# nextpyp/pyp

Measured on AMD Instinct MI355X. Metric: particles/sec projection-matching, 256^2 box, higher is better.
Workload: dtype f32

## Files before the change

### pyp_amd/csrc/host_refine.h

```cpp
#pragma once

static int launch_prep(DevBuf<float2> &spill , const float *d_images, const double *d_rows, int n_img, const Geom &gm, double Rm_px, float fall_px,
                       int normalize, int invert, int do_mask, int whiten, float2 *band, float *wring,
                       const uint32_t *samples, int S_pad, float2 *Il, float *cw, float2 *Wp, float *C2, float *nI,
                       unsigned *band_max = nullptr ,
                       const float *focus_px = nullptr ) {
    if (int rc = ensure_plan(gm.N)) return rc;
    PrepP P;
    P.images = d_images; P.rows = d_rows; P.plan = g.plans[gm.N].plan;
    P.N = gm.N; P.B = gm.B; P.W = gm.W; P.H = gm.H;
    P.r_hi2 = (float)(gm.r_hi * gm.r_hi); P.Rm = (float)Rm_px; P.wfall = fall_px; P.a = (float)gm.a;
    P.Rm2_bg = (float)std::min(std::floor(Rm_px * Rm_px), 16777216.0);
    P.normalize = normalize; P.invert = invert; P.do_mask = do_mask; P.whiten = whiten;
    for (int k = 0; k < 4; k++) P.focus[k] = focus_px ? focus_px[k] : 0.f;
    P.band_max = band_max;
    P.band = band; P.wring = wring; P.samples = samples; P.S_pad = S_pad; P.Il = Il; P.cw = cw;
    P.Wp = Wp; P.C2 = C2; P.nI = nI; P.Bs = gm.Bs; P.Hs = gm.Hs;
    P.r_s2 = (float)(gm.r_s * gm.r_s); P.r_lo2 = (float)(gm.r_lo * gm.r_lo);
    const PrepPlan pl = prep_plan(gm.N, gm.B, gm.W);
    if (pl.err) return fail(-12, pl.err);
    P.L = pl.L; P.nc = pl.nc; P.nchunks = pl.nchunks; P.TS = pl.TS; P.WS = pl.WS;
    P.spill = nullptr;
    if (!pl.scratch_free) {
        if (int rc = spill.ensure((size_t)n_img * gm.N * gm.W)) return rc;
        P.spill = spill.p;
    }
    if (int rc = pl.scratch_free ? raise_lds_limit((const void *)k_prep<512, 2>, 160 * 1024) : raise_lds_limit((const void *)k_prep<256, 3>, 80 * 1024)) return rc;
    ProfScope ps(PPM_K_PREP);
    if (pl.scratch_free) hipLaunchKernelGGL((k_prep<512, 2>), dim3(n_img), dim3(512), pl.lds.total, cur_stream(), P);
    else hipLaunchKernelGGL((k_prep<256, 3>), dim3(n_img), dim3(256), pl.lds.total, cur_stream(), P);
    HIPCHK(hipGetLastError());
    return 0;
}

template <int... I>
static const void *global_kernel_at(int i, std::integer_sequence<int, I...>) {
    static const void *const fn[] = { (const void *)k_global<I / 4 + 1, (I & 2) != 0, (I & 1) != 0>... };
    return fn[i];
}
static const void *global_kernel(int R, bool half, int Bs) {
    const bool two = Bs <= 31;
    return global_kernel_at(((R >= 1 && R <= 5 ? R : 6) - 1) * 4 + (half ? 2 : 0) + (two ? 1 : 0), std::make_integer_sequence<int, 24>());
}
static size_t global_lds_bytes(int HsP, int n_orient, int R, int *topk_lds) {
    size_t lds = (size_t)HsP * 64 * sizeof(float2) * global_particles(R);
    if (lds < 1024) lds = 1024;
    const size_t lds_topk = (size_t)(32 + n_orient) * sizeof(float);
    const int fits = lds_topk <= (size_t)160 * 1024 ? 1 : 0;
    if (topk_lds) *topk_lds = fits;
    if (fits && lds_topk > lds) lds = lds_topk;
    return lds;
}
static int launch_global(GlobP &P, int n_img, bool half, int R) {
    P.n = n_img;
    const size_t lds = global_lds_bytes(P.HsP, P.n_orient, R, &P.topk_lds);
    const void *fn = global_kernel(R, half, P.Bs);
    if (int rc = raise_lds_limit(fn, 160 * 1024)) return rc;
    ProfScope ps(PPM_K_GLOBAL);
    const int ngroups = (n_img + global_particles(R) - 1) / global_particles(R);
    void *args[] = { &P };
    HIPCHK(hipLaunchKernel(fn, dim3(std::min(ngroups, g.cu_count)), dim3(global_threads(R)), args, lds, cur_stream()));
    return 0;
}

struct GfftPlan { int LN = 0, L = 0, RC = 0, nchunk = 1; size_t fixed = 0, t_bytes = 0, lds = 0; int topk_lds = 0; };
static bool gfft_plan(const Geom &gm, GfftPlan &pl) {
    int LN = 0; while ((1 << LN) < gm.Ns) LN++;
    if ((1 << LN) != gm.Ns || LN < 4 || LN > 7) return false;
    pl.LN = LN; pl.L = gm.Ns / 2;
    const int L = pl.L, G = gfft_slices_per_pass(L), NR = 2 * gm.RSy + 1;
    const size_t row = (size_t)G * 2 * gfft_row_stride(L) * sizeof(float2), fixed = (size_t)L * L * sizeof(float4) + gfft_small_bytes(L);
    const size_t room = (size_t)160 * 1024 - fixed;
    int RC = NR;
    if (const char *e = getenv("PPM_GFFT_ROWS")) { const int v = atoi(e); if (v > 0 && v < RC) RC = v; }
    if ((size_t)RC * row > room) RC = (int)(room / row);
    if (RC > 2 * L) RC = 2 * L;
    pl.RC = RC; pl.nchunk = (NR + RC - 1) / RC;
    pl.RC = (NR + pl.nchunk - 1) / pl.nchunk;
    pl.t_bytes = std::max((size_t)pl.RC * row, (size_t)G * L * L * sizeof(float4));
    pl.fixed = fixed;
    return true;
}
static void gfft_plan_topk(GfftPlan &pl, int n_orient) {
    const size_t topk = (size_t)n_orient * sizeof(float);
    pl.topk_lds = 0;
    if (topk <= pl.t_bytes) pl.topk_lds = 1;
    else if (pl.fixed + topk <= (size_t)160 * 1024) { pl.topk_lds = 1; pl.t_bytes = (topk + 15) & ~(size_t)15; }
    pl.lds = pl.fixed + pl.t_bytes;
}
static const void *gfft_kernel(int LN, bool chunked) {
    static const void *const fn[] = { (const void *)k_gfft<4, false>, (const void *)k_gfft<4, true>, (const void *)k_gfft<5, false>, (const void *)k_gfft<5, true>,
                                      (const void *)k_gfft<6, false>, (const void *)k_gfft<6, true>, (const void *)k_gfft<7, false>, (const void *)k_gfft<7, true> };
    return fn[((LN >= 4 && LN <= 6 ? LN : 7) - 4) * 2 + (chunked ? 1 : 0)];
}
static int launch_gfft(GfftP &P, int n_img, const GfftPlan &pl) {
    P.n = n_img; P.RC = pl.RC; P.nchunk = pl.nchunk; P.t_bytes = (int)pl.t_bytes; P.topk_lds = pl.topk_lds;
    const void *fn = gfft_kernel(pl.LN, pl.nchunk > 1);
    if (int rc = raise_lds_limit(fn, 160 * 1024)) return rc;
    ProfScope ps(PPM_K_GLOBAL);
    void *args[] = { &P };
    HIPCHK(hipLaunchKernel(fn, dim3(n_img), dim3(256), args, pl.lds, cur_stream()));
#ifdef PPM_GFFT_STAMPS
    {
        float st[4 * 4 * 12];
        HIPCHK(hipStreamSynchronize(cur_stream()));
        HIPCHK(hipMemcpy(st, P.cc, sizeof(st), hipMemcpyDeviceToHost));
        const char *names[12] = { "products", "fft", "stores", "barrier A", "row tail", "barrier B", "twiddles", "loop", "row reads + pairs", "row fft", "row max", "-" };
        const int nsl = P.n_dir * P.npsi_store;
        for (int b = 0; b < 4 && b < n_img; b++) for (int w = 0; w < 4; w++) {
            fprintf(stderr, "k_gfft stamps block %d wave %d (cycles per slice):", b, w);
            for (int i = 0; i < 11; i++) fprintf(stderr, " | %s %.0f", names[i], st[(b * 4 + w) * 12 + i] / nsl);
            fprintf(stderr, "\n");
        }
    }
#endif
    return 0;
}

static void launch_defocus(const CubeView &cv, const Geom &gm, const uint32_t *samples, int S_pad, const float2 *Il, const float *wring, const double *rows,
                           LState *states, int n, int nt, float step, float *ddef, double *all_scores, float rcls2) {
    const int nrings = gm.B + 2;
    DefocusP DP;
    DP.cv = cv; DP.samples = samples; DP.Il = Il; DP.wring = wring; DP.S_pad = S_pad; DP.nrings = nrings; DP.N = gm.N; DP.B = gm.B;
    DP.rlo2 = (float)(gm.r_lo * gm.r_lo); DP.rmax2 = (float)(gm.r_hi * gm.r_hi); DP.ring_signed = (float)std::min(gm.ring_signed, 1e30); DP.a = (float)gm.a;
    DP.rows = rows; DP.states = states; DP.ddef = ddef; DP.nt = nt; DP.step = step; DP.all_scores = all_scores; DP.rcls2 = rcls2;
    long knob = 0;
    if (const char *e = std::getenv("PPM_DEFOCUS_CHUNK")) knob = std::atol(e);
    DP.tchunk = ppm::defocus_chunk(nt, nrings, knob);
    ProfScope ps(PPM_K_LOCAL);
    hipLaunchKernelGGL(k_defocus, dim3(n), dim3(256), ring_lds_bytes(4, DP.tchunk, nrings), cur_stream(), DP);
}

namespace {
struct LocalLaunch { LocalP P = {}; int threads = 0, per_particle = 1; double evals = 0; bool near = false; };
struct RefineRun {
    ppm_ref *ref = nullptr; const ppm_refine_cfg *cfg = nullptr;
    Geom gm; SampleList sl; CubeView cv;
    int S_pad = 0, nrings = 0, CH = 0;
    int K = 0, Tb = 0, Tc = 0;
    double Rm_px = 0; float fall_px = 0;
    bool focus_on = false, sep_search = false; float focus_px[4] = { 0, 0, 0, 0 };
    GfftPlan gpl; bool use_fft = false;
    RowPlan rows = {};
    int Rtx = 0, Rty = 0, Rwin = 0, HsP = 0, nslices = 0; std::vector<int> cxs, cys;
    std::vector<GridSection> secs; std::vector<int> kpre; int sec_dirs = 0;
    LocalP base = {}; bool local_tab = false;
    double bf = 3.0; bool any_ang = false, any_sh = false;
    double ha0 = 0, hs0 = 0;
    int ndef = 0;
    int per_iter = 0; bool cls_on = false;
    LocalLaunch hit, fin;
    double sample_evals = 0;
    bool overlap = false; int tenants = 0;
    unsigned long long *reuse = nullptr;

    int ntiles() const { return (int)(cxs.size() * cys.size()); }
    int nsec() const { return (int)secs.size(); }
    size_t bank_slice() const { return (size_t)HsP * 64; }
    size_t bank4_slice() const { return use_fft ? (size_t)gpl.L * gpl.L : 0; }
    size_t HS() const { return (size_t)gm.Hs * 64; }
    int prefix_of(double rband) const { int rg = (int)std::ceil(rband); if (rg > gm.B + 1) rg = gm.B + 1; return sl.ring_off[rg]; }
    int reach_of(int S) const { int b = gm.B + 2; while (b > 1 && sl.ring_off[b] > S) b--; return std::min(gm.B, b - 1); }
};
constexpr int kTileR = 6;
constexpr int kFinalThreads = 256;
}

static void refine_notes(ppm_ref *ref, const ppm_refine_cfg *cfg, const Geom &gm) {
    ref->note.clear();
    if (gm.r_s_asked > gm.r_s) {
        char b[256];
        std::snprintf(b, sizeof(b), "NOTE: global search band lowered from %.1f to %.1f Fourier pixels (%.2f A instead of %.2f A): the grid-search "
                      "kernel covers 64 pixels; the top hits are refined up to the high-resolution limit as asked", gm.r_s_asked, gm.r_s,
                      gm.N * gm.a / gm.r_s, gm.N * gm.a / gm.r_s_asked);
        ref->note = b;
    }
    if (cfg->global_search && gm.range_capped) {
        char b[320];
        std::snprintf(b, sizeof(b), "%sNOTE: shift window of the grid search: +-%.0f x +-%.0f pixels (%d x %d search-grid steps of %.1f pixels, the most the "
                      "search grid of %d points holds; asked: %.0f pixels); the refinement of the hits is not limited to it", ref->note.empty() ? "" : "\n",
                      gm.RSx * gm.step, gm.RSy * gm.step, gm.RSx, gm.RSy, gm.step, gm.Ns, gm.range_asked_px);
        ref->note += b;
    }
}

static size_t workspace_budget() { return g.total_mem / 4; }
static size_t bank_budget() {
    size_t b = g.total_mem / 4;
    if (const char *e = std::getenv("PPM_BANK_BYTES")) { const long long v = std::atoll(e); if (v > 0 && (size_t)v < b) b = (size_t)v; }
    return b;
}

static int plan_grid_sections(RefineRun &r) {
    ppm_ref *ref = r.ref; const Geom &gm = r.gm;
    std::string err;
    const size_t budget = bank_budget();
    if (!plan_sections(gm.n_dir, gm.npsi_store, r.bank_slice() * sizeof(float2), r.bank4_slice() * sizeof(float4), budget, r.secs, err)) return fail(-22, err);
    if (r.nsec() > 1 && !r.use_fft && r.ntiles() > 1) {
        char b[320];
        std::snprintf(b, sizeof(b), "PPM_GLOBAL_PATH=tiles keeps the slice bank of the whole grid (%.2f GB at an angular step of %.3g degrees), the bank may take "
                      "%.2f GB; use a coarser angular step or the default path, which searches the grid in sections", (double)r.nslices * r.bank_slice() * sizeof(float2) / 1073741824.0,
                      gm.dstep, budget / 1073741824.0);
        return fail(-22, b);
// ... 706 lines not shown
```

### pyp_amd/csrc/ppm_kernels.h

```cpp
#pragma once
#include "ppm_dev.h"
#include "ppm_geom.h"
#include "ppm_rows.h"
#include "ppm_window.h"
#include <type_traits>

namespace ppm {

struct FftLinesP {
    float2 *data; FftPlan plan;
    int n, inverse, line_major, L;
    long nlines, inner, inner_stride, outer_stride, elem_stride;
};

__global__ void __launch_bounds__(256) k_fft_lines(FftLinesP P) {
    extern __shared__ __attribute__((aligned(16))) char smem[];
    __shared__ long lbase[16];
    __shared__ float2 tw_s[512];
    float2 *buf = (float2 *)smem;
    const int tid = threadIdx.x, n = P.n, LS = n + 1;
    long l0 = (long)blockIdx.x * P.L;
    int nl = (int)((P.nlines - l0) < P.L ? (P.nlines - l0) : P.L);
    if (nl <= 0) return;
    if (tid < nl) { const long l = l0 + tid; lbase[tid] = (l / P.inner) * P.outer_stride + (l % P.inner) * P.inner_stride; }
    for (int i = tid; i < n; i += 256) tw_s[i] = P.plan.tw[i];
    __syncthreads();
    const int dl = P.line_major ? 256 % nl : 256 / n, de = P.line_major ? 256 / nl : 256 % n;
    const int line0 = P.line_major ? tid % nl : tid / n, e0 = P.line_major ? tid / nl : tid % n;
    auto next = [&](int &line, int &e) {
        line += dl; e += de;
        if (P.line_major) { if (line >= nl) { line -= nl; e++; } } else if (e >= n) { e -= n; line++; }
    };
    {
        int line = line0, e = e0;
        for (int i = tid; i < nl * n; i += 256, next(line, e)) buf[line * LS + P.plan.perm[e]] = P.data[lbase[line] + e * P.elem_stride];
    }
    lds_fft(buf, P.plan, nl, LS, P.inverse != 0, tid, 256, tw_s);
    {
        int line = line0, e = e0;
        for (int i = tid; i < nl * n; i += 256, next(line, e)) P.data[lbase[line] + e * P.elem_stride] = buf[line * LS + e];
    }
}

__global__ void k_ref_load(const float *__restrict__ vol, float2 *__restrict__ f, int n, int np) {
    size_t i = (size_t)blockIdx.x * blockDim.x + threadIdx.x, n3 = (size_t)n * n * n;
    if (i >= n3) return;
    int x = (int)(i % n), y = (int)((i / n) % n), z = (int)(i / ((size_t)n * n));
    float g = 1.f;
    int c[3] = { x, y, z };
#pragma unroll
    for (int q = 0; q < 3; q++) {
        float u = kPiF * (float)(c[q] - n / 2) / (float)np;
        float sv = fabsf(u) < 1e-6f ? 1.f : sinf(u) / u;
        g *= 1.f / (sv * sv);
    }
    const int o0 = (np - n) / 2;
    f[((size_t)(z + o0) * np + (y + o0)) * np + (x + o0)] = make_float2(vol[i] * g, 0.f);
}

__global__ void k_ref_crop(const float2 *__restrict__ f, float2 *__restrict__ cube, int n, int n_orig, int B, int CX, int CY, int NBX, int NBY, unsigned LB,
                           const float *__restrict__ ringw, int nw) {
    size_t i = (size_t)blockIdx.x * blockDim.x + threadIdx.x, tot = (size_t)CX * CY * CY;
    if (i >= tot) return;
    const int x = (int)(i % CX), ys = (int)((i / CX) % CY), zs = (int)(i / ((size_t)CX * CY));
    const int y = ys - (B + 1), z = zs - (B + 1);
    int iz = ((z % n) + n) % n, iy = ((y % n) + n) % n, ix = x % n;
    float2 v = f[((size_t)iz * n + iy) * n + ix];
    float sg = (((x + y + z) & 1) ? -1.f : 1.f) / (float)n_orig;
    if (ringw) {
        const float kk = sqrtf((float)(x * x + y * y + z * z)) * (float)n_orig / (float)n;
        const int k0 = (int)kk;
        const float fr = kk - (float)k0;
        sg *= k0 + 1 < nw ? ringw[k0] + fr * (ringw[k0 + 1] - ringw[k0]) : ringw[nw - 1];
    }
    v = make_float2(v.x * sg, v.y * sg);
    cube[cube_element(NBX, NBY, LB, 0, x, ys, zs)] = v;
    if (x >= 2) cube[cube_element(NBX, NBY, LB, 1, x, ys, zs)] = v;
}

struct PrepP {
    const float *images; const double *rows; FftPlan plan;
    int N, B, W, H;
    float r_hi2, Rm, wfall, a;
    float Rm2_bg;
    float focus[4];
    int normalize, invert, do_mask, whiten;
    int nc, nchunks, L;
    int TS, WS;
    float2 *band;
    unsigned *band_max;
    float2 *spill;
    float *wring;
    const uint32_t *samples; int S_pad; float2 *Il; float *cw;
    float2 *Wp; float *C2; float *nI; int Bs, Hs; float r_s2, r_lo2;
};

template <int PT>
struct PrepBlock {
    static constexpr int PW = PT / 64;
    static constexpr bool kScratchFree = PT == 512;
    const PrepP &P;
    const int tid, p, N, B, W, H, TS, WS;
    const float *img; float2 *bandp;
    float2 *T, *Wk; unsigned long long *ringq; unsigned *ringc; float *ringpw; double *red; float *stat, *fmask; float2 *tw_s;
    unsigned short *perm_s, *iperm_s;
    double s1 = 0, s2 = 0, cnt = 0, t1 = 0, t2 = 0;
    float mu = 0.f, sc = 1.f, qscale = 1.f, oscale = 1.f;
    float mcx = 0.f, mcy = 0.f, mrad = 0.f, wf;
    float btx = 0.f, bty = 0.f; bool beam_tilt = false;
    float omax = 0.f;

    __device__ __forceinline__ PrepBlock(const PrepP &P_, char *smem)
        : P(P_), tid(threadIdx.x), p(blockIdx.x), N(P_.N), B(P_.B), W(P_.W), H(P_.H), TS(P_.TS), WS(P_.WS),
          img(P_.images + (size_t)blockIdx.x * P_.N * P_.N), bandp(P_.band + (size_t)blockIdx.x * P_.H * P_.W), wf(P_.wfall < 1e-3f ? 1e-3f : P_.wfall) {
        const PrepLds l = prep_lds(kScratchFree, N, B, P.L, P.nc, TS, WS);
        T = (float2 *)(smem + l.T.off); Wk = (float2 *)(smem + l.Wk.off);
        ringq = (unsigned long long *)(smem + l.ringq.off); ringc = (unsigned *)(smem + l.ringc.off); ringpw = (float *)(smem + l.ringpw.off);
        red = (double *)(smem + l.red.off); stat = (float *)(smem + l.stat.off); fmask = (float *)(smem + l.fmask.off);
        tw_s = (float2 *)(smem + l.tw.off); perm_s = (unsigned short *)(smem + l.perm.off); iperm_s = (unsigned short *)(smem + l.iperm.off);
    }

    __device__ __forceinline__ void background_stats() {
        const float Rm2 = P.Rm2_bg;
        const float invNf = 1.0f / (float)N;
        const float4 *img4 = (const float4 *)img;
        constexpr int UR = 8;
        const bool rows4 = (N & 3) == 0;
        for (int b4 = tid; b4 < N * N / 4; b4 += PT * UR) {
            float4 qv[UR];
#pragma unroll
            for (int u = 0; u < UR; u++) { const int i4 = b4 + u * PT; if (i4 < N * N / 4) qv[u] = img4[i4]; }
            float f1 = 0.f, f2 = 0.f, fc = 0.f, g1 = 0.f, g2 = 0.f;
#pragma unroll
            for (int u = 0; u < UR; u++) {
                const int i4 = b4 + u * PT;
                if (i4 >= N * N / 4) continue;
                const float vv[4] = { qv[u].x, qv[u].y, qv[u].z, qv[u].w };
                const int i0 = 4 * i4, y0 = fast_div(i0, N, invNf), x0 = i0 - y0 * N;
#pragma unroll
                for (int j = 0; j < 4; j++) {
                    int y = y0, x = x0 + j;
                    if (!rows4 && x >= N) { x -= N; y += 1; }
                    const float dx = (float)(x - N / 2), dy = (float)(y - N / 2), v = vv[j];
                    g1 += v; g2 = fmaf(v, v, g2);
                    if (dx * dx + dy * dy > Rm2) { f1 += v; f2 = fmaf(v, v, f2); fc += 1.f; }
                }
            }
            s1 += (double)f1; s2 += (double)f2; cnt += (double)fc; t1 += (double)g1; t2 += (double)g2;
        }
    }

    __device__ __forceinline__ void finish_stats() {
        s1 = wave_sum_d(s1); s2 = wave_sum_d(s2); cnt = wave_sum_d(cnt); t1 = wave_sum_d(t1); t2 = wave_sum_d(t2);
        if ((tid & 63) == 0) { int w = tid >> 6; red[w * 4] = s1; red[w * 4 + 1] = s2; red[w * 4 + 2] = cnt; red[w * 4 + 3] = t1; }
        __syncthreads();
        if (tid == 0) {
            double a1 = 0, a2 = 0, ac = 0, b1 = 0;
// ... 450 lines not shown
    for (int k = 0; k < K; k++) {
        int bt = -1, bj = -1; float bc = -3.0e38f; int bo = 0x7fffffff;
        for (int t = 0; t < ntiles; t++) {
            const Hit *h = tiles + ((size_t)t * n + p) * K;
            for (int j = 0; j < K; j++) {
                if (h[j].orient < 0) continue;
                if (h[j].cc > bc || (h[j].cc == bc && h[j].orient < bo)) { bc = h[j].cc; bo = h[j].orient; bt = t; bj = j; }
            }
        }
        Hit o; o.cc = 0.f; o.orient = 0; o.sx = 0; o.sy = 0;
        if (bt >= 0) {
            o = tiles[((size_t)bt * n + p) * K + bj];
            o.sx += cx[bt]; o.sy += cy[bt];
            for (int t = 0; t < ntiles; t++) {
                Hit *h = tiles + ((size_t)t * n + p) * K;
                for (int j = 0; j < K; j++) if (h[j].orient == bo) h[j].orient = -1;
            }
        }
        out[(size_t)p * K + k] = o;
    }
}

__global__ void __launch_bounds__(64) k_merge_sections(const Hit *lists, Hit *out, int n, int K, int nsec, const int *kpre) {
    const int p = blockIdx.x, lane = threadIdx.x;
    for (int s = 0; s < nsec; s++) {
        const int k0 = kpre[s], ks = kpre[s + 1] - k0;
        if (lane >= ks) continue;
        const Hit me = lists[(size_t)k0 * n + (size_t)p * ks + lane];
        const int mi = k0 + lane;
        int rank = 0;
        for (int t = 0; t < nsec && rank < K; t++) {
            const int t0 = kpre[t], kt = kpre[t + 1] - t0;
            const Hit *h = lists + (size_t)t0 * n + (size_t)p * kt;
            for (int j = 0; j < kt; j++) {
                const float c = h[j].cc; const int o = h[j].orient;
                rank += (c > me.cc || (c == me.cc && (o < me.orient || (o == me.orient && t0 + j < mi)))) ? 1 : 0;
            }
        }
        if (rank < K) out[(size_t)p * K + rank] = me;
    }
}

constexpr int kRowTwRows = 64;
#ifndef PPM_GLOBAL_PARTICLES
#define PPM_GLOBAL_PARTICLES 2
#endif
#ifndef PPM_GLOBAL_PAIR_MAXR
#define PPM_GLOBAL_PAIR_MAXR 8
#endif
#ifndef PPM_GLOBAL_THREADS
#define PPM_GLOBAL_THREADS 512
#endif
#ifndef PPM_GLOBAL_UNROLL
#define PPM_GLOBAL_UNROLL 4
#endif
#ifndef PPM_GLOBAL_FOLD
#define PPM_GLOBAL_FOLD 1
#endif
constexpr bool global_fold(int Bs) { return PPM_GLOBAL_FOLD != 0 && Bs > 31; }
typedef float v2f __attribute__((ext_vector_type(2)));
typedef float v4f __attribute__((ext_vector_type(4)));
typedef const __attribute__((address_space(4))) v4f *RowTwPtr;

struct GlobP {
    const float2 *bank; const float2 *Wp; const float *nP; const float *nI; const float2 *twN;
    const float4 *rowtw;
    float *cc; int *sh;
    Hit *hits;
    int n, Bs, Hs, HsP, Ns, RSx, RSy, n_dir, n_psi, npsi_store, n_orient, K;
    int topk_lds;
    int nP_ld, o_ld, o_base;
    RowPlan rows;
};

template <int M> __device__ __forceinline__ v2f halve_pair2(v2f a, v2f b, int lane) {
    float a0 = a.x, a1 = a.y, b0 = b.x, b1 = b.y;
    if constexpr (M >= 16) {
        lane_swap<M>(a0, b0); lane_swap<M>(a1, b1);
        return (v2f){ a0, a1 } + (v2f){ b0, b1 };
    } else {
        constexpr int ctrl = M == 8 ? kDppRor8 : M == 4 ? kDppHalfMirror : M == 2 ? kDppXor2 : kDppXor1;
        const bool hi = (lane & M) != 0;
        const float t0 = a0 + dpp_mov<ctrl>(a0), t1 = a1 + dpp_mov<ctrl>(a1), u0 = b0 + dpp_mov<ctrl>(b0), u1 = b1 + dpp_mov<ctrl>(b1);
        return (v2f){ hi ? u0 : t0, hi ? u1 : t1 };
    }
}
template <int NV>
__device__ __forceinline__ v2f reduce_halving2(v2f (&v)[NV], int lane) {
    static_assert(NV <= 64, "one output register pair");
    constexpr int n1 = (NV + 1) / 2, n2 = (n1 + 1) / 2, n3 = (n2 + 1) / 2, n4 = (n3 + 1) / 2, n5 = (n4 + 1) / 2;
    const v2f z = { 0.f, 0.f };
    v2f a1[n1], a2[n2], a3[n3], a4[n4], a5[n5];
#pragma unroll
    for (int i = 0; i < n1; i++) a1[i] = halve_pair2<32>(v[2 * i], (2 * i + 1 < NV) ? v[2 * i + 1] : z, lane);
#pragma unroll
    for (int i = 0; i < n2; i++) a2[i] = halve_pair2<16>(a1[2 * i], (2 * i + 1 < n1) ? a1[2 * i + 1] : z, lane);
#pragma unroll
    for (int i = 0; i < n3; i++) a3[i] = halve_pair2<8>(a2[2 * i], (2 * i + 1 < n2) ? a2[2 * i + 1] : z, lane);
#pragma unroll
    for (int i = 0; i < n4; i++) a4[i] = halve_pair2<4>(a3[2 * i], (2 * i + 1 < n3) ? a3[2 * i + 1] : z, lane);
#pragma unroll
    for (int i = 0; i < n5; i++) a5[i] = halve_pair2<2>(a4[2 * i], (2 * i + 1 < n4) ? a4[2 * i + 1] : z, lane);
    return halve_pair2<1>(a5[0], (n5 > 1) ? a5[1] : z, lane);
}

template <int NV>
__device__ __forceinline__ v2f reduce_halving2h(v2f (&v)[NV], int lane) {
    static_assert(NV <= 32, "one output register pair per half");
    constexpr int n2 = (NV + 1) / 2, n3 = (n2 + 1) / 2, n4 = (n3 + 1) / 2, n5 = (n4 + 1) / 2;
    const v2f z = { 0.f, 0.f };
    v2f a2[n2], a3[n3], a4[n4], a5[n5];
#pragma unroll
    for (int i = 0; i < n2; i++) a2[i] = halve_pair2<16>(v[2 * i], (2 * i + 1 < NV) ? v[2 * i + 1] : z, lane);
#pragma unroll
    for (int i = 0; i < n3; i++) a3[i] = halve_pair2<8>(a2[2 * i], (2 * i + 1 < n2) ? a2[2 * i + 1] : z, lane);
#pragma unroll
    for (int i = 0; i < n4; i++) a4[i] = halve_pair2<4>(a3[2 * i], (2 * i + 1 < n3) ? a3[2 * i + 1] : z, lane);
#pragma unroll
    for (int i = 0; i < n5; i++) a5[i] = halve_pair2<2>(a4[2 * i], (2 * i + 1 < n4) ? a4[2 * i + 1] : z, lane);
    return halve_pair2<1>(a5[0], (n5 > 1) ? a5[1] : z, lane);
}

constexpr int global_particles(int R) { return R <= PPM_GLOBAL_PAIR_MAXR ? PPM_GLOBAL_PARTICLES : 1; }
constexpr int global_threads(int R) { return R <= 3 ? PPM_GLOBAL_THREADS : 512; }
constexpr int global_unroll(int R) { return R <= 3 ? PPM_GLOBAL_UNROLL : 4; }

template <int M> __device__ __forceinline__ float halve_pair(float a, float b, int lane) {
    if constexpr (M >= 16) { lane_swap<M>(a, b); return a + b; }
    else {
        constexpr int ctrl = M == 8 ? kDppRor8 : M == 4 ? kDppHalfMirror : M == 2 ? kDppXor2 : kDppXor1;
        const float t = a + dpp_mov<ctrl>(a), u = b + dpp_mov<ctrl>(b);
        return (lane & M) ? u : t;
    }
}

template <int NV>
__device__ __forceinline__ float reduce_halving(float (&v)[NV], int lane) {
    static_assert(NV <= 64, "one output register");
    constexpr int n1 = (NV + 1) / 2, n2 = (n1 + 1) / 2, n3 = (n2 + 1) / 2, n4 = (n3 + 1) / 2, n5 = (n4 + 1) / 2;
    float a1[n1], a2[n2], a3[n3], a4[n4], a5[n5];
#pragma unroll
    for (int i = 0; i < n1; i++) a1[i] = halve_pair<32>(v[2 * i], (2 * i + 1 < NV) ? v[2 * i + 1] : 0.f, lane);
#pragma unroll
    for (int i = 0; i < n2; i++) a2[i] = halve_pair<16>(a1[2 * i], (2 * i + 1 < n1) ? a1[2 * i + 1] : 0.f, lane);
#pragma unroll
    for (int i = 0; i < n3; i++) a3[i] = halve_pair<8>(a2[2 * i], (2 * i + 1 < n2) ? a2[2 * i + 1] : 0.f, lane);
#pragma unroll
    for (int i = 0; i < n4; i++) a4[i] = halve_pair<4>(a3[2 * i], (2 * i + 1 < n3) ? a3[2 * i + 1] : 0.f, lane);
#pragma unroll
    for (int i = 0; i < n5; i++) a5[i] = halve_pair<2>(a4[2 * i], (2 * i + 1 < n4) ? a4[2 * i + 1] : 0.f, lane);
    return halve_pair<1>(a5[0], (n5 > 1) ? a5[1] : 0.f, lane);
}

template <int R, bool HALF, bool TWO>
__global__ void __launch_bounds__(global_threads(R)) k_global(GlobP P) {
    constexpr int NT = global_threads(R), NW = NT / 64, U = global_unroll(R), NS = 2 * R + 1, NQ = global_particles(R);
    extern __shared__ __attribute__((aligned(16))) char smem[];
    const int tid = threadIdx.x, lane = tid & 63;
    const int sub = TWO ? lane >> 5 : 0, kxl = TWO ? lane & 31 : lane;
    const int wave = __builtin_amdgcn_readfirstlane(tid >> 6);
    const int Hs = P.Hs, HsP = P.HsP, Bs = P.Bs, Ns = P.Ns, nsampP = HsP * 64;
    const int nslices = P.n_dir * P.npsi_store;
    constexpr bool kFold = !TWO && PPM_GLOBAL_FOLD != 0;
    static_assert(!kFold || U == 4, "a step is one quad of rows");
    const int plain_rows = kFold ? 4 * P.rows.plain_steps : HsP;
    float2 *Wl = (float2 *)smem;
    constexpr bool kXFold = !TWO && HALF && NS * NS <= 64;
    const int kxt = kXFold ? lane & 31 : kxl;
    float txc[R + 1], txs[R + 1];
#pragma unroll
    for (int j = 0; j <= R; j++) {
        float2 t = P.twN[(kxt * j) & (Ns - 1)];
        txc[j] = t.x; txs[j] = t.y;
    }
    const RowTwPtr c_rowtw = (RowTwPtr)P.rowtw;
    const int ngroups = (P.n + NQ - 1) / NQ;
    for (int grp = blockIdx.x; grp < ngroups; grp += gridDim.x) {
    const int p0 = grp * NQ;
    int pq[NQ];
#pragma unroll
    for (int q = 0; q < NQ; q++) pq[q] = min(p0 + q, P.n - 1);
#pragma unroll
    for (int q = 0; q < NQ; q++) {
        const float2 *src = P.Wp + (size_t)pq[q] * Hs * 64;
        for (int i = tid; i < nsampP; i += NT) {
            int ky = 0;
            const bool ok = row_ky(P.rows, i >> 6, ky);
            const int srow = ky + Bs;
            Wl[q * nsampP + i] = ok ? src[srow * 64 + (i & 63)] : make_float2(0.f, 0.f);
        }
    }
    __syncthreads();
    float nI[NQ];
    const __attribute__((address_space(4))) float *c_nP[NQ];
#pragma unroll
    for (int q = 0; q < NQ; q++) {
        nI[q] = P.nI[pq[q]];
        c_nP[q] = (const __attribute__((address_space(4))) float *)P.nP + (size_t)pq[q] * P.nP_ld;
    }
    float2 pv[U], pn[U];
    const int nsl = TWO ? (nslices + 1) / 2 : nslices;
    auto my_slice = [&](int s) { return TWO ? min(2 * s + sub, nslices - 1) : s; };
    if (wave < nsl) {
        const float2 *P0 = P.bank + (size_t)my_slice(wave) * nsampP;
#pragma unroll
        for (int u = 0; u < U; u++) pv[u] = P0[u * 64 + kxl];
    }
    for (int sl = wave; sl < nsl; sl += NW) {
        const int msl = my_slice(sl);
        const bool live = !TWO || 2 * sl + sub < nslices;
        const float2 *Pp = P.bank + (size_t)msl * nsampP;
        const float2 *Pnext = P.bank + (size_t)my_slice(sl + NW < nsl ? sl + NW : sl) * nsampP;
        constexpr bool kSetFirst = R <= 3;
        v2f sa[NQ], sb[NQ], ua[NQ][R], ub[NQ][R], va[NQ][R], vb[NQ][R];
        if constexpr (!kSetFirst) {
#pragma unroll
            for (int q = 0; q < NQ; q++) {
                sa[q] = sb[q] = (v2f){ 0.f, 0.f };
#pragma unroll
                for (int j = 0; j < R; j++) { ua[q][j] = ub[q][j] = va[q][j] = vb[q][j] = (v2f){ 0.f, 0.f }; }
            }
        }
        auto step = [&](auto first, int row0, const float2 (&cur)[U], float2 (&nxt)[U]) {
            constexpr bool kFirst = decltype(first)::value;
            {
                const float2 *np = (row0 + U < HsP) ? Pp + (row0 + U) * 64 : Pnext;
#pragma unroll
                for (int u = 0; u < U; u++) nxt[u] = np[u * 64 + kxl];
            }
            v4f tw[R], twn[R];
#pragma unroll
            for (int j = 0; j < R; j++) tw[j] = c_rowtw[(row0 >> 1) * PPM_MAX_SHIFT_STEPS + j];
            float2 wa[NQ], wb[NQ];
#pragma unroll
            for (int q = 0; q < NQ; q++) { wa[q] = Wl[q * nsampP + row0 * 64 + kxl]; wb[q] = Wl[q * nsampP + (row0 + 1) * 64 + kxl]; }
#pragma unroll
            for (int u = 0; u < U; u += 2) {
                const int ra = row0 + u, tp = ra >> 1;
                float2 wan[NQ], wbn[NQ];
#pragma unroll
                for (int q = 0; q < NQ; q++) { wan[q] = wa[q]; wbn[q] = wb[q]; }
                if (u + 2 < U) {
#pragma unroll
                    for (int j = 0; j < R; j++) twn[j] = c_rowtw[(tp + 1) * PPM_MAX_SHIFT_STEPS + j];
#pragma unroll
                    for (int q = 0; q < NQ; q++) { wan[q] = Wl[q * nsampP + (ra + 2) * 64 + kxl]; wbn[q] = Wl[q * nsampP + (ra + 3) * 64 + kxl]; }
                }
                const float pax = cur[u].x, pay = cur[u].y, pbx = cur[u + 1].x, pby = cur[u + 1].y;
#pragma unroll
                for (int q = 0; q < NQ; q++) {
                    const v2f wav = { wa[q].x, wa[q].y }, wbv = { wb[q].x, wb[q].y };
                    const v2f aa = wav * pax, ab = wbv * pbx, ba = wav * pay, bb = wbv * pby;
                    const v2f as2 = aa + ab, ad2 = aa - ab, bs2 = ba + bb, bd2 = ba - bb;
                    if (kFirst && u == 0) { sa[q] = as2; sb[q] = bs2; } else { sa[q] += as2; sb[q] += bs2; }
#pragma unroll
                    for (int j = 0; j < R; j++) {
                        const v4f t = tw[j];
                        const v2f tc = { t.x, t.y }, ts = { t.z, t.w };
                        if (kFirst && u == 0) {
                            ua[q][j] = as2 * tc; ub[q][j] = bs2 * tc;
                            va[q][j] = ad2 * ts; vb[q][j] = bd2 * ts;
                        } else {
                            ua[q][j] += as2 * tc; ub[q][j] += bs2 * tc;
                            va[q][j] += ad2 * ts; vb[q][j] += bd2 * ts;
                        }
                    }
                }
#pragma unroll
                for (int j = 0; j < R; j++) tw[j] = twn[j];
#pragma unroll
                for (int q = 0; q < NQ; q++) { wa[q] = wan[q]; wb[q] = wbn[q]; }
            }
        };
        auto qstep = [&](int row0, const float2 (&cur)[U], float2 (&nxt)[U]) {
            {
                const float2 *np = (row0 + U < HsP) ? Pp + (row0 + U) * 64 : Pnext;
#pragma unroll
                for (int u = 0; u < U; u++) nxt[u] = np[u * 64 + kxl];
            }
            v4f tw[R];
#pragma unroll
            for (int j = 0; j < R; j++) tw[j] = c_rowtw[(row0 >> 1) * PPM_MAX_SHIFT_STEPS + j];
            float2 w[NQ][U];
#pragma unroll
            for (int q = 0; q < NQ; q++)
#pragma unroll
                for (int u = 0; u < U; u++) w[q][u] = Wl[q * nsampP + (row0 + u) * 64 + kxl];
#pragma unroll
            for (int q = 0; q < NQ; q++) {
                v2f as2[2], ad2[2], bs2[2], bd2[2];
#pragma unroll
                for (int h = 0; h < 2; h++) {
                    const v2f wav = { w[q][2 * h].x, w[q][2 * h].y }, wbv = { w[q][2 * h + 1].x, w[q][2 * h + 1].y };
                    const v2f aa = wav * cur[2 * h].x, ab = wbv * cur[2 * h + 1].x, ba = wav * cur[2 * h].y, bb = wbv * cur[2 * h + 1].y;
                    as2[h] = aa + ab; ad2[h] = aa - ab; bs2[h] = ba + bb; bd2[h] = ba - bb;
                }
                const v2f ea[2] = { as2[0] + as2[1], as2[0] - as2[1] }, eb[2] = { bs2[0] + bs2[1], bs2[0] - bs2[1] };
                const v2f oa[2] = { ad2[0] - ad2[1], ad2[0] + ad2[1] }, ob[2] = { bd2[0] - bd2[1], bd2[0] + bd2[1] };
                sa[q] += ea[0]; sb[q] += eb[0];
#pragma unroll
                for (int j = 0; j < R; j++) {
                    const v4f t = tw[j];
                    const v2f tc = { t.x, t.y }, ts = { t.z, t.w };
                    const int par = (j + 1) & 1;
                    ua[q][j] += ea[par] * tc; ub[q][j] += eb[par] * tc;
                    va[q][j] += oa[par] * ts; vb[q][j] += ob[par] * ts;
                }
            }
        };
        __builtin_amdgcn_s_setprio(3);
        constexpr std::true_type kSets = {}; constexpr std::false_type kAdds = {};
        int row0 = 0;
        if constexpr (kSetFirst) {
            step(kSets, 0, pv, pn);
            if (!kFold || 2 * U <= plain_rows) step(kAdds, U, pn, pv);
            else qstep(U, pn, pv);
            row0 = 2 * U;
        }
        for (; row0 + 2 * U <= plain_rows; row0 += 2 * U) { step(kAdds, row0, pv, pn); step(kAdds, row0 + U, pn, pv); }
        if constexpr (kFold) {
            if (row0 < plain_rows) { step(kAdds, row0, pv, pn); qstep(row0 + U, pn, pv); row0 += 2 * U; }
            for (; row0 < HsP; row0 += 2 * U) { qstep(row0, pv, pn); qstep(row0 + U, pn, pv); }
        }
        __builtin_amdgcn_s_setprio(0);
        const int dir = msl / P.npsi_store, ks = msl - dir * P.npsi_store;
#pragma unroll
        for (int q = 0; q < NQ; q++) {
            const float nP = c_nP[q][msl];
            const float sax = sa[q].x, say = sa[q].y, sbx = sb[q].y, sby = -sb[q].x;
            float uax[R], uay[R], ubx[R], uby[R], vax[R], vay[R], vbx[R], vby[R];
#pragma unroll
            for (int j = 0; j < R; j++) {
                uax[j] = ua[q][j].x; uay[j] = ua[q][j].y; ubx[j] = ub[q][j].y; uby[j] = -ub[q][j].x;
                vax[j] = va[q][j].x; vay[j] = va[q][j].y; vbx[j] = vb[q][j].y; vby[j] = -vb[q][j].x;
            }
            const float inv = (nP > 0.f && nI[q] > 0.f) ? rsqrtf(nP * nI[q]) : 0.f;
            float *ccp = P.cc + (size_t)pq[q] * P.o_ld; int *shp = P.sh + (size_t)pq[q] * P.o_ld;
            if constexpr (!TWO && HALF && NS * NS <= 64) {
                const v2f sg2 = { 1.f, -1.f };
                constexpr int NV = win_values(R);
                v2f gxr[NS], gyr[NS], val[NV];
#pragma unroll
                for (int iy = 0; iy < NS; iy++) {
// ... 6 lines not shown
                    }
                }
#pragma unroll
                for (int s = 0; s < win_slots(R); s++) {
                    const int ra = 2 * s, rb = ra + 1 < NS ? ra + 1 : ra;
                    float ax0 = gxr[ra].x, ax1 = gxr[ra].y, ay0 = gyr[ra].x, ay1 = gyr[ra].y;
                    float bx0 = gxr[rb].x, bx1 = gxr[rb].y, by0 = gyr[rb].x, by1 = gyr[rb].y;
                    lane_swap<32>(ax0, bx0); lane_swap<32>(ax1, bx1); lane_swap<32>(ay0, by0); lane_swap<32>(ay1, by1);
                    const v2f gx = { ax0, ax1 }, gy = { ay0, ay1 }, hx = { bx0, bx1 }, hy = { by0, by1 };
                    const v2f Sx = gx + hx, Dx = gx - hx, Dy = gy - hy, Px = gx - hy, Py = gy + hx, Qx = gx + hy, Qy = gy - hx;
                    val[s * NS + R] = Sx;
#pragma unroll
                    for (int j = 1; j <= R; j++) {
                        static_assert(R <= 3, "j = 4 would take S_y");
                        if (j == 2) {
                            const v2f pc = Dx * txc[j], qs = Dy * txs[j];
                            val[s * NS + R + j] = pc - qs;
                            val[s * NS + R - j] = pc + qs;
                        } else {
                            const v2f &px = j == 1 ? Px : Qx, &py = j == 1 ? Py : Qy, &mx = j == 1 ? Qx : Px, &my = j == 1 ? Qy : Py;
                            val[s * NS + R + j] = px * txc[j] - py * txs[j];
                            val[s * NS + R - j] = mx * txc[j] + my * txs[j];
                        }
                    }
                }
                const v2f tot = reduce_halving2h<NV>(val, lane);
                int iy = 0, ix = 0;
                const bool inwin = win_valid(R, win_lane_value(lane), win_lane_half(lane), P.RSx, P.RSy, iy, ix);
                const int vi = win_key(R, iy, ix);
#pragma unroll
                for (int e = 0; e < 2; e++) {
                    const float cand = inwin ? (e ? tot.y : tot.x) : -3.0e38f;
                    const float best = wave_max(cand);
                    int ci = wave_min(cand == best && inwin ? vi : 64);
                    if (ci > 63) ci = 0;
                    const int bsy_ = ci / NS - R, bsx_ = ci - (ci / NS) * NS - R;
                    if (lane == 0 && (q == 0 || p0 + q < P.n)) {
                        int o = dir * P.n_psi + ks + e * P.npsi_store;
                        ccp[o] = best * inv;
                        shp[o] = (bsx_ & 0xffff) | (bsy_ << 16);
                    }
                }
            } else if constexpr (TWO || NS * NS > 64) {
                const v2f sg2 = { 1.f, -1.f };
                const int vi = TWO ? (int)(__brev((unsigned)kxl) >> 27) : (int)(__brev((unsigned)lane) >> 26), ix = vi;
                const int ax = ix - R < 0 ? R - ix : ix - R;
                const bool incol = vi < NS && ax <= P.RSx;
                float bestv[2] = { -3.0e38f, -3.0e38f }; int besty[2] = { 0, 0 };
#pragma unroll
                for (int iy = 0; iy < NS; iy++) {
                    const int jy = iy - R, ja = jy < 0 ? -jy : jy;
                    v2f gx, gy;
                    if (jy == 0) { gx = sax + sg2 * sbx; gy = say + sg2 * sby; }
                    else {
                        const v2f ux = uax[ja - 1] + sg2 * ubx[ja - 1], uy = uay[ja - 1] + sg2 * uby[ja - 1];
                        const v2f vx = vax[ja - 1] + sg2 * vbx[ja - 1], vy = vay[ja - 1] + sg2 * vby[ja - 1];
                        gx = jy > 0 ? ux - vy : ux + vy; gy = jy > 0 ? uy + vx : uy - vx;
                    }
                    v2f val[NS];
                    val[R] = gx;
#pragma unroll
                    for (int j = 1; j <= R; j++) {
                        const v2f pc = gx * txc[j], qs = gy * txs[j];
                        val[R + j] = pc - qs;
                        val[R - j] = pc + qs;
                    }
                    v2f tot;
                    if constexpr (TWO) tot = reduce_halving2h<NS>(val, lane); else tot = reduce_halving2<NS>(val, lane);
                    const bool ok = incol && ja <= P.RSy;
#pragma unroll
                    for (int e = 0; e < (HALF ? 2 : 1); e++) {
                        const float cand = ok ? (e ? tot.y : tot.x) : -3.0e38f;
                        if (cand > bestv[e]) { bestv[e] = cand; besty[e] = iy; }
                    }
                }
#pragma unroll
                for (int e = 0; e < (HALF ? 2 : 1); e++) {
                    const float best = TWO ? half_max(bestv[e]) : wave_max(bestv[e]);
                    const int key = bestv[e] == best ? besty[e] * NS + vi : 1 << 20;
                    int ci = TWO ? half_min(key) : wave_min(key);
                    if (ci >= NS * NS) ci = R * NS + R;
                    const int bsy_ = ci / NS - R, bsx_ = ci - (ci / NS) * NS - R;
                    if (kxl == 0 && live && (q == 0 || p0 + q < P.n)) {
                        int o = dir * P.n_psi + ks + e * P.npsi_store;
                        ccp[o] = best * inv;
                        shp[o] = (bsx_ & 0xffff) | (bsy_ << 16);
                    }
                }
            } else
#pragma unroll
            for (int e = 0; e < (HALF ? 2 : 1); e++) {
                const float sg = e ? -1.f : 1.f;
                float best = -3.0e38f; int bsx_ = 0, bsy_ = 0;
                if constexpr (NS * NS <= 64) {
                    float val[NS * NS];
#pragma unroll
                    for (int iy = 0; iy < NS; iy++) {
                        const int jy = iy - R, ja = jy < 0 ? -jy : jy;
                        float gx, gy;
                        if (jy == 0) { gx = sax + sg * sbx; gy = say + sg * sby; }
                        else {
                            const float ux = uax[ja - 1] + sg * ubx[ja - 1], uy = uay[ja - 1] + sg * uby[ja - 1];
                            const float vx = vax[ja - 1] + sg * vbx[ja - 1], vy = vay[ja - 1] + sg * vby[ja - 1];
                            gx = jy > 0 ? ux - vy : ux + vy; gy = jy > 0 ? uy + vx : uy - vx;
                        }
                        val[iy * NS + R] = gx;
#pragma unroll
                        for (int j = 1; j <= R; j++) {
                            const float pc = gx * txc[j], qs = gy * txs[j];
                            val[iy * NS + R + j] = pc - qs;
                            val[iy * NS + R - j] = pc + qs;
                        }
                    }
                    const float tot = reduce_halving<NS * NS>(val, lane);
                    const int vi = (int)(__brev((unsigned)lane) >> 26);
                    const int iy = vi / NS, ix = vi - iy * NS;
                    const int ay = iy - R < 0 ? R - iy : iy - R, ax = ix - R < 0 ? R - ix : ix - R;
                    const float cand = (vi < NS * NS && ax <= P.RSx && ay <= P.RSy) ? tot : -3.0e38f;
                    best = wave_max(cand);
                    int ci = wave_min(cand == best ? vi : 64);
                    if (ci > 63) ci = 0;
                    bsy_ = ci / NS - R; bsx_ = ci - (ci / NS) * NS - R;
                } else {
#pragma unroll
                    for (int iy = 0; iy < NS; iy++) {
                        const int jy = iy - R, ja = jy < 0 ? -jy : jy;
                        float gx, gy;
                        if (jy == 0) { gx = sax + sg * sbx; gy = say + sg * sby; }
                        else {
                            const float ux = uax[ja - 1] + sg * ubx[ja - 1], uy = uay[ja - 1] + sg * uby[ja - 1];
                            const float vx = vax[ja - 1] + sg * vbx[ja - 1], vy = vay[ja - 1] + sg * vby[ja - 1];
                            gx = jy > 0 ? ux - vy : ux + vy; gy = jy > 0 ? uy + vx : uy - vx;
                        }
#pragma unroll
                        for (int ix = 0; ix < NS; ix++) {
                            const int j = ix - R, jx = j < 0 ? -j : j;
                            float v = j >= 0 ? (gx * txc[jx] - gy * txs[jx]) : (gx * txc[jx] + gy * txs[jx]);
                            v = wave_sum(v);
                            bool ok = (jx <= P.RSx) && (ja <= P.RSy);
                            if (ok && v > best) { best = v; bsx_ = j; bsy_ = jy; }
                        }
                    }
                }
                if (lane == 0 && (q == 0 || p0 + q < P.n)) {
                    int o = dir * P.n_psi + ks + e * P.npsi_store;
                    ccp[o] = best * inv;
                    shp[o] = (bsx_ & 0xffff) | (bsy_ << 16);
                }
            }
        }
    }
    __threadfence_block();
    __syncthreads();
    float *rv = (float *)smem; int *ri = (int *)(rv + 16);
    for (int q = 0; q < NQ && p0 + q < P.n; q++) {
        const int p = p0 + q;
        float *ccp = P.cc + (size_t)p * P.o_ld; int *shp = P.sh + (size_t)p * P.o_ld;
        float *sc = P.topk_lds ? rv + 32 : ccp;
        if (P.topk_lds) for (int o = tid; o < P.n_orient; o += NT) sc[o] = ccp[o];
        __syncthreads();
        for (int k = 0; k < P.K; k++) {
            float bv = -3.0e38f; int bi = 0x7fffffff;
            for (int o = tid; o < P.n_orient; o += NT) {
                const float v = sc[o];
                if (v > bv || (v == bv && o < bi)) { bv = v; bi = o; }
            }
#pragma unroll
            for (int m = 32; m >= 1; m >>= 1) {
                float ov = __shfl_xor(bv, m, 64); int oi = __shfl_xor(bi, m, 64);
                if (ov > bv || (ov == bv && oi < bi)) { bv = ov; bi = oi; }
            }
            if (lane == 0) { rv[wave] = bv; ri[wave] = bi; }
            __syncthreads();
            if (tid == 0) {
                for (int w = 1; w < NW; w++) if (rv[w] > bv || (rv[w] == bv && ri[w] < bi)) { bv = rv[w]; bi = ri[w]; }
                if (bi >= P.n_orient) { bi = 0; bv = 0.f; }
                Hit h; h.cc = bv; h.orient = bi + P.o_base;
                int sv = shp[bi];
                h.sx = (int)(short)(sv & 0xffff); h.sy = sv >> 16;
                P.hits[(size_t)p * P.K + k] = h;
                if (bi < P.n_orient) sc[bi] = -__builtin_inff();
            }
            __threadfence_block();
            __syncthreads();
        }
    }
    __syncthreads();
    }
}

}
```

Before: 95030.

## Run per-particle top-K selection in single waves with LDS copies, batch Wp staging

The top-K hit extraction changes from block-wide passes with a __syncthreads per rank to one wave per particle. Each wave scans an LDS copy of the scores padded to 1024-entry rows, uses float4 loads and a DPP/lane-swap reduction, and writes all K hits at the end. LDS sizing now holds several particle copies at once. The Wp staging loop is also restructured so each wave loads 8 rows for all particles into registers before storing them to LDS. This removes many block barriers and serial tid-0 work, at the cost of more LDS, more registers, and new DPP helper code.

Result: no change. 94980, median of 2 (-0.1%).

```diff
diff --git a/pyp_amd/csrc/host_refine.h b/pyp_amd/csrc/host_refine.h
--- a/pyp_amd/csrc/host_refine.h
+++ b/pyp_amd/csrc/host_refine.h
@@ -45,10 +45,10 @@
 static size_t global_lds_bytes(int HsP, int n_orient, int R, int *topk_lds) {
     size_t lds = (size_t)HsP * 64 * sizeof(float2) * global_particles(R);
     if (lds < 1024) lds = 1024;
-    const size_t lds_topk = (size_t)(32 + n_orient) * sizeof(float);
-    const int fits = lds_topk <= (size_t)160 * 1024 ? 1 : 0;
-    if (topk_lds) *topk_lds = fits;
-    if (fits && lds_topk > lds) lds = lds_topk;
+    const size_t copy = (size_t)std::max(topk_padded(n_orient), topk_row()) * sizeof(float);
+    const int copies = (int)std::min<size_t>((size_t)160 * 1024 / copy, (size_t)global_particles(R));
+    if (topk_lds) *topk_lds = copies;
+    if (copies * copy > lds) lds = copies * copy;
     return lds;
 }
 static int launch_global(GlobP &P, int n_img, bool half, int R) {
diff --git a/pyp_amd/csrc/ppm_kernels.h b/pyp_amd/csrc/ppm_kernels.h
--- a/pyp_amd/csrc/ppm_kernels.h
+++ b/pyp_amd/csrc/ppm_kernels.h
@@ -3,6 +3,7 @@
 #include "ppm_geom.h"
 #include "ppm_rows.h"
 #include "ppm_window.h"
+#include "ppm_topk.h"
 #include <type_traits>
 
 namespace ppm {
@@ -759,6 +760,17 @@
     return halve_pair<1>(a5[0], (n5 > 1) ? a5[1] : 0.f, lane);
 }
 
+__device__ __forceinline__ void wave_topk_best(float &bv, int &bi) {
+    topk_take(dpp_mov<kDppXor1>(bv), dpp_mov<kDppXor1>(bi), bv, bi);
+    topk_take(dpp_mov<kDppXor2>(bv), dpp_mov<kDppXor2>(bi), bv, bi);
+    topk_take(dpp_mov<kDppHalfMirror>(bv), dpp_mov<kDppHalfMirror>(bi), bv, bi);
+    topk_take(dpp_mov<kDppMirror>(bv), dpp_mov<kDppMirror>(bi), bv, bi);
+    float wv = bv; int wi = bi;
+    lane_swap<16>(bv, wv); lane_swap<16>(bi, wi); topk_take(wv, wi, bv, bi);
+    wv = bv; wi = bi;
+    lane_swap<32>(bv, wv); lane_swap<32>(bi, wi); topk_take(wv, wi, bv, bi);
+}
+
 template <int R, bool HALF, bool TWO>
 __global__ void __launch_bounds__(global_threads(R)) k_global(GlobP P) {
     constexpr int NT = global_threads(R), NW = NT / 64, U = global_unroll(R), NS = 2 * R + 1, NQ = global_particles(R);
@@ -787,15 +799,37 @@
     int pq[NQ];
 #pragma unroll
     for (int q = 0; q < NQ; q++) pq[q] = min(p0 + q, P.n - 1);
-#pragma unroll
-    for (int q = 0; q < NQ; q++) {
-        const float2 *src = P.Wp + (size_t)pq[q] * Hs * 64;
-        for (int i = tid; i < nsampP; i += NT) {
+    constexpr int kStageRows = 8;
+    auto stage_rows = [&](auto whole, int r0) {
+        constexpr bool kWhole = decltype(whole)::value;
+        int srow[kStageRows];
+#pragma unroll
+        for (int b = 0; b < kStageRows; b++) {
+            const int r = r0 + b * NW;
             int ky = 0;
-            const bool ok = row_ky(P.rows, i >> 6, ky);
-            const int srow = ky + Bs;
-            Wl[q * nsampP + i] = ok ? src[srow * 64 + (i & 63)] : make_float2(0.f, 0.f);
-        }
+            srow[b] = (kWhole || r < HsP) && row_ky(P.rows, r, ky) ? ky + Bs : -1;
+        }
+        float2 w[kStageRows][NQ];
+#pragma unroll
+        for (int b = 0; b < kStageRows; b++)
+#pragma unroll
+            for (int q = 0; q < NQ; q++) {
+                w[b][q] = make_float2(0.f, 0.f);
+                if (srow[b] >= 0) w[b][q] = P.Wp[((size_t)pq[q] * Hs + srow[b]) * 64 + lane];
+            }
+#pragma unroll
+        for (int b = 0; b < kStageRows; b++) {
+            const int r = r0 + b * NW;
+            if (kWhole || r < HsP) {
+#pragma unroll
+                for (int q = 0; q < NQ; q++) Wl[q * nsampP + r * 64 + lane] = w[b][q];
+            }
+        }
+    };
+    {
+        int r0 = wave;
+        for (; r0 + (kStageRows - 1) * NW < HsP; r0 += NW * kStageRows) stage_rows(std::true_type{}, r0);
+        if (r0 < HsP) stage_rows(std::false_type{}, r0);
     }
     __syncthreads();
     float nI[NQ];
@@ -1108,37 +1142,89 @@
     }
     __threadfence_block();
     __syncthreads();
-    float *rv = (float *)smem; int *ri = (int *)(rv + 16);
-    for (int q = 0; q < NQ && p0 + q < P.n; q++) {
-        const int p = p0 + q;
-        float *ccp = P.cc + (size_t)p * P.o_ld; int *shp = P.sh + (size_t)p * P.o_ld;
-        float *sc = P.topk_lds ? rv + 32 : ccp;
-        if (P.topk_lds) for (int o = tid; o < P.n_orient; o += NT) sc[o] = ccp[o];
-        __syncthreads();
-        for (int k = 0; k < P.K; k++) {
-            float bv = -3.0e38f; int bi = 0x7fffffff;
-            for (int o = tid; o < P.n_orient; o += NT) {
-                const float v = sc[o];
-                if (v > bv || (v == bv && o < bi)) { bv = v; bi = o; }
-            }
-#pragma unroll
-            for (int m = 32; m >= 1; m >>= 1) {
-                float ov = __shfl_xor(bv, m, 64); int oi = __shfl_xor(bi, m, 64);
-                if (ov > bv || (ov == bv && oi < bi)) { bv = ov; bi = oi; }
-            }
-            if (lane == 0) { rv[wave] = bv; ri[wave] = bi; }
+    if (P.topk_lds > 0) {
+        static_assert(PPM_MAX_TOP_HITS <= 64, "lane k keeps rank k");
+        const int ncopy = min(P.topk_lds, NQ), npad = topk_padded(P.n_orient);
+        float *scl = (float *)smem;
+        for (int q0 = 0; q0 < NQ && p0 + q0 < P.n; q0 += ncopy) {
+            if (q0) __syncthreads();
+            constexpr int kCopyBatch = 8;
+            for (int c = 0; c < ncopy && q0 + c < NQ && p0 + q0 + c < P.n; c++) {
+                const float *ccp = P.cc + (size_t)(p0 + q0 + c) * P.o_ld;
+                float *sc = scl + c * npad;
+                for (int ob = tid; ob < npad; ob += NT * kCopyBatch) {
+                    float v[kCopyBatch];
+#pragma unroll
+                    for (int b = 0; b < kCopyBatch; b++) {
+                        const int o = ob + b * NT;
+                        v[b] = topk_struck();
+                        if (o < P.n_orient) v[b] = ccp[o];
+                    }
+#pragma unroll
+                    for (int b = 0; b < kCopyBatch; b++) {
+                        const int o = ob + b * NT;
+                        if (o < npad) sc[o] = v[b];
+                    }
+                }
+            }
             __syncthreads();
-            if (tid == 0) {
-                for (int w = 1; w < NW; w++) if (rv[w] > bv || (rv[w] == bv && ri[w] < bi)) { bv = rv[w]; bi = ri[w]; }
-                if (bi >= P.n_orient) { bi = 0; bv = 0.f; }
-                Hit h; h.cc = bv; h.orient = bi + P.o_base;
-                int sv = shp[bi];
-                h.sx = (int)(short)(sv & 0xffff); h.sy = sv >> 16;
-                P.hits[(size_t)p * P.K + k] = h;
-                if (bi < P.n_orient) sc[bi] = -__builtin_inff();
-            }
-            __threadfence_block();
-            __syncthreads();
+            if (wave < ncopy && q0 + wave < NQ && p0 + q0 + wave < P.n) {
+                const int p = p0 + q0 + wave;
+                float *sc = scl + wave * npad;
+                float kv = 0.f; int ko = 0;
+                for (int k = 0; k < P.K; k++) {
+                    float bv = topk_start_value(); int bi = topk_start_index();
+                    for (int row = npad / topk_row() - 1; row >= 0; row--) {
+                        float4 v[topk_row_parts()];
+#pragma unroll
+                        for (int c = 0; c < topk_row_parts(); c++) v[c] = *(const float4 *)(sc + topk_lane_first(row, c, lane));
+#pragma unroll
+                        for (int c = topk_row_parts() - 1; c >= 0; c--) {
+                            const int o = topk_lane_first(row, c, lane);
+                            topk_take_descending(v[c].w, o + 3, bv, bi); topk_take_descending(v[c].z, o + 2, bv, bi);
+                            topk_take_descending(v[c].y, o + 1, bv, bi); topk_take_descending(v[c].x, o, bv, bi);
+                        }
+                    }
+                    wave_topk_best(bv, bi);
+                    topk_settle(P.n_orient, bv, bi);
+                    if (lane == k) { kv = bv; ko = bi; }
+                    if (lane == 0) sc[bi] = topk_struck();
+                }
+                if (lane < P.K) {
+                    const int sv = P.sh[(size_t)p * P.o_ld + ko];
+                    Hit h; h.cc = kv; h.orient = ko + P.o_base;
+                    h.sx = (int)(short)(sv & 0xffff); h.sy = sv >> 16;
+                    P.hits[(size_t)p * P.K + lane] = h;
+                }
+            }
+        }
+    } else {
+        float *rv = (float *)smem; int *ri = (int *)(rv + 16);
+        for (int q = 0; q < NQ && p0 + q < P.n; q++) {
+            const int p = p0 + q;
+            float *sc = P.cc + (size_t)p * P.o_ld; int *shp = P.sh + (size_t)p * P.o_ld;
+            for (int k = 0; k < P.K; k++) {
+                float bv = topk_start_value(); int bi = topk_start_index();
+                for (int o = tid; o < P.n_orient; o += NT) topk_take(sc[o], o, bv, bi);
+#pragma unroll
+                for (int m = 32; m >= 1; m >>= 1) {
+                    const float ov = __shfl_xor(bv, m, 64); const int oi = __shfl_xor(bi, m, 64);
+                    topk_take(ov, oi, bv, bi);
+                }
+                if (lane == 0) { rv[wave] = bv; ri[wave] = bi; }
+                __syncthreads();
+                if (tid == 0) {
+                    for (int w = 1; w < NW; w++) topk_take(rv[w], ri[w], bv, bi);
+                    topk_settle(P.n_orient, bv, bi);
+                    Hit h; h.cc = bv; h.orient = bi + P.o_base;
+                    int sv = shp[bi];
+                    h.sx = (int)(short)(sv & 0xffff); h.sy = sv >> 16;
+                    P.hits[(size_t)p * P.K + k] = h;
+                    sc[bi] = topk_struck();
+                }
+                __threadfence_block();
+                __syncthreads();
+            }
         }
     }
     __syncthreads();
diff --git a/pyp_amd/csrc/ppm_topk.h b/pyp_amd/csrc/ppm_topk.h
--- /dev/null
+++ b/pyp_amd/csrc/ppm_topk.h
@@ -0,0 +1,34 @@
+#pragma once
+
+#ifndef PPM_HD
+#ifdef __HIPCC__
+#define PPM_HD __host__ __device__
+#else
+#define PPM_HD
+#endif
+#endif
+
+namespace ppm {
+
+PPM_HD constexpr float topk_start_value() { return -3.0e38f; }
+PPM_HD constexpr int topk_start_index() { return 0x7fffffff; }
+PPM_HD inline float topk_struck() { return -__builtin_inff(); }
+
+PPM_HD inline bool topk_better(float v, int i, float bv, int bi) { return v > bv || (v == bv && i < bi); }
+PPM_HD inline void topk_take(float v, int i, float &bv, int &bi) {
+    if (topk_better(v, i, bv, bi)) { bv = v; bi = i; }
+}
+PPM_HD inline void topk_take_descending(float v, int i, float &bv, int &bi) {
+    if (v >= bv) { bv = v; bi = i; }
+}
+
+PPM_HD inline void topk_settle(int n_orient, float &bv, int &bi) {
+    if (bi >= n_orient) { bi = 0; bv = 0.f; }
+}
+
+PPM_HD constexpr int topk_row_parts() { return 4; }
+PPM_HD constexpr int topk_row() { return topk_row_parts() * 256; }
+PPM_HD constexpr int topk_padded(int n_orient) { return (n_orient + topk_row() - 1) / topk_row() * topk_row(); }
+PPM_HD constexpr int topk_lane_first(int row, int part, int lane) { return row * topk_row() + part * 256 + 4 * lane; }
+
+}
```
